# mistralai/mistral-inference

Measured on NVIDIA H100. Metric: decode tokens/sec (bf16, batch=1, seq=4k) [+ prefill TFLOPS, both vs roofline], higher is better.
Workload: dtype bf16

## Files before the change

mistral_inference_b200/csrc/abi.cu:

```cuda
#include <cmath>
#include <cstdlib>
#include <cstring>

#include "attn_decode_tma.cuh"
#include "attn_full_hd64.cuh"
#include "attn_prefill.cuh"
#include "attn_prefill_wgmma.cuh"
#include "decode_megakernel.cuh"
#include "elementwise.cuh"
#include "gemm_mma.cuh"
#include "gemm_streamk.cuh"
#include "gemm_wgmma.cuh"
#include "kv_fp8.cuh"
#include "lora.cuh"
#include "moe.cuh"
#include "sampling.cuh"
#include "skinny_linear.cuh"
#include "vision.cuh"
#include "workspace.cuh"

namespace mb200 {
thread_local char g_err[512] = "";
thread_local bool g_launch_log_on = false;
thread_local bool g_launch_log_overflow = false;
// ... 854 lines not shown
  MB_CHECK_ARG((size_t)sms * sizeof(unsigned long long) <= kWsMkArgmaxSlots.bytes, "decode_step: %d SMs exceed the argmax slots", sms);
  uint8_t* ws = (uint8_t*)workspace;
  p.argmax_counter = (int*)(ws + kWsMkArgmaxCounter.offset);
  p.argmax_slots = (unsigned long long*)(ws + kWsMkArgmaxSlots.offset);
  p.bar_flags = (unsigned*)(ws + kWsMkBarFlags.offset);
  p.bar_epoch = (unsigned*)(ws + kWsMkBarEpoch.offset);
  p.done_counter = (int*)(ws + kWsMkDoneCounter.offset);
  const DecodeScratch sc = decode_scratch(dim, hidden, n_heads, n_experts, top_k, sms);
  p.xbuf = (bf16*)(ws + sc.xbuf);
  p.hbuf = (bf16*)(ws + sc.hbuf);
  p.qbuf = (bf16*)(ws + sc.qbuf);
  p.abuf = (bf16*)(ws + sc.abuf);
  p.gbuf = (bf16*)(ws + sc.gbuf);
  p.partial = (float*)(ws + sc.partial);
  p.prof = g_mk_prof;
  p.prof_bar = g_mk_prof_bar;
  if (workspace_bytes < sc.end) return fail(MB200_E_WORKSPACE, "decode_step: workspace %zu < %zu", workspace_bytes, sc.end);

  void* args[] = {(void*)&p};
  const void* fn = nullptr;
  switch (rep) {
    case 1: fn = w8 ? (const void*)decode_megakernel<1, true> : (const void*)decode_megakernel<1>; break;
    case 2: fn = w8 ? (const void*)decode_megakernel<2, true> : (const void*)decode_megakernel<2>; break;
    case 4: fn = w8 ? (const void*)decode_megakernel<4, true> : (const void*)decode_megakernel<4>; break;
    case 6: fn = w8 ? (const void*)decode_megakernel<6, true> : (const void*)decode_megakernel<6>; break;
    case 8: fn = w8 ? (const void*)decode_megakernel<8, true> : (const void*)decode_megakernel<8>; break;
    default: return fail(MB200_E_INVALID, "decode_step: H/KV=%d unsupported (1,2,4,6,8)", rep);
  }
  if (w8)
    note_launch("decode_megakernel<%d, true>", rep);
  else
    note_launch("decode_megakernel<%d>", rep);
  MB_CHECK_CUDA(cudaFuncSetAttribute(fn, cudaFuncAttributeMaxDynamicSharedMemorySize, (int)smem));
  MB_CHECK_CUDA(cudaLaunchCooperativeKernel(fn, dim3((unsigned)sms), dim3(MK_THREADS), args, smem, (cudaStream_t)stream));
  return MB200_OK;
}

extern "C" {

int mb200_decode_step(const mb200_layer_desc* layers_dev, const int32_t* windows_dev, int64_t n_layers, const void* emb, const void* final_norm,
                      const void* w_out, const float* rope, const int64_t* token_dev, int64_t pos, int64_t batch_row, float* logits,
                      int64_t* next_token_dev, int64_t dim,
                      int64_t hidden, int64_t n_heads, int64_t n_kv_heads, int64_t head_dim, int64_t vocab, float eps, int64_t n_experts,
                      int64_t top_k, const void* const* moe_gate_dev, const void* const* moe_w13_dev, const void* const* moe_w2_dev,
                      void* workspace, size_t workspace_bytes, void* stream) {
  return decode_step_impl(layers_dev, windows_dev, n_layers, emb, final_norm, w_out, rope, token_dev, pos, batch_row, logits, next_token_dev, dim,
                          hidden, n_heads, n_kv_heads, head_dim, vocab, eps, n_experts, top_k, moe_gate_dev, moe_w13_dev, moe_w2_dev, workspace,
                          workspace_bytes, stream, false);
}

int mb200_decode_step_fp8(const mb200_layer_desc_fp8* layers_dev, const int32_t* windows_dev, int64_t n_layers, const void* emb,
                          const void* final_norm, const void* w_out, const float* rope, const int64_t* token_dev, int64_t pos,
                          int64_t batch_row, float* logits, int64_t* next_token_dev, int64_t dim, int64_t hidden, int64_t n_heads,
                          int64_t n_kv_heads, int64_t head_dim, int64_t vocab, float eps, void* workspace, size_t workspace_bytes, void* stream) {
  return decode_step_impl(layers_dev, windows_dev, n_layers, emb, final_norm, w_out, rope, token_dev, pos, batch_row, logits, next_token_dev, dim,
                          hidden, n_heads, n_kv_heads, head_dim, vocab, eps, 0, 0, nullptr, nullptr, nullptr, workspace, workspace_bytes, stream,
                          true);
}

int mb200_decode_step_fp8_supported(int64_t dim, int64_t hidden, int64_t n_heads, int64_t n_kv_heads, int64_t head_dim, int64_t vocab,
                                    int64_t smem_optin) {
  if (smem_optin <= 0) {
    int dev = 0, smem_max = 0;
    MB_CHECK_CUDA(cudaGetDevice(&dev));
    MB_CHECK_CUDA(cudaDeviceGetAttribute(&smem_max, cudaDevAttrMaxSharedMemoryPerBlockOptin, dev));
    smem_optin = smem_max;
  }
  DecodePlan plan;
  return decode_plan(dim, hidden, n_heads, n_kv_heads, head_dim, vocab, 0, 0, smem_optin, &plan, true);
}

int mb200_debug_decode_scratch(int64_t dim, int64_t hidden, int64_t n_heads, int64_t n_kv_heads, int64_t head_dim, int64_t n_experts,
                               int64_t top_k, size_t* q_offset, size_t* attn_offset) {
  MB_CHECK_ARG(q_offset && attn_offset, "debug_decode_scratch: null pointer");
  size_t off[6];
  const int rc = mb200_debug_decode_buffers(dim, hidden, n_heads, n_kv_heads, head_dim, n_experts, top_k, off);
  if (rc) return rc;
  *q_offset = off[2];
  *attn_offset = off[3];
  return MB200_OK;
}

int mb200_debug_decode_buffers(int64_t dim, int64_t hidden, int64_t n_heads, int64_t n_kv_heads, int64_t head_dim, int64_t n_experts,
                               int64_t top_k, size_t* offsets) {
  MB_CHECK_ARG(offsets, "debug_decode_buffers: null pointer");
  MB_CHECK_ARG(head_dim == kHeadDim && n_kv_heads > 0 && n_heads % n_kv_heads == 0 && dim > 0 && hidden > 0,
               "debug_decode_scratch: bad shape (H=%lld, KV=%lld, hd=%lld)", (long long)n_heads, (long long)n_kv_heads, (long long)head_dim);
  const DecodeScratch sc = decode_scratch(dim, hidden, n_heads, n_experts, top_k, 0);
  offsets[0] = sc.xbuf;
  offsets[1] = sc.hbuf;
  offsets[2] = sc.qbuf;
  offsets[3] = sc.abuf;
  offsets[4] = sc.gbuf;
  offsets[5] = sc.partial;
  return MB200_OK;
}

int mb200_decode_step_supported(int64_t dim, int64_t hidden, int64_t n_heads, int64_t n_kv_heads, int64_t head_dim, int64_t vocab,
                                int64_t n_experts, int64_t top_k, int64_t smem_optin) {
  if (smem_optin <= 0) {
    int dev = 0, smem_max = 0;
    MB_CHECK_CUDA(cudaGetDevice(&dev));
    MB_CHECK_CUDA(cudaDeviceGetAttribute(&smem_max, cudaDevAttrMaxSharedMemoryPerBlockOptin, dev));
    smem_optin = smem_max;
  }
  DecodePlan plan;
  return decode_plan(dim, hidden, n_heads, n_kv_heads, head_dim, vocab, n_experts, top_k, smem_optin, &plan);
}

int mb200_debug_set_decode_timeline(void* device_buffer) {
  g_mk_prof = (unsigned long long*)device_buffer;
  return MB200_OK;
}
int mb200_debug_set_barrier_timeline(void* device_buffer) {
  g_mk_prof_bar = (unsigned long long*)device_buffer;
  return MB200_OK;
}

int mb200_debug_launch_log(int enable, char* out, size_t out_bytes) {
  const bool overflow = g_launch_log_overflow;
  const size_t len = g_launch_log_len;
  g_launch_log_on = enable != 0;
  g_launch_log_overflow = false;
  g_launch_log_len = 0;
  if (out != nullptr) {
    if (out_bytes < len + 1) return fail(MB200_E_INVALID, "launch log: %zu bytes recorded, buffer of %zu", len, out_bytes);
    memcpy(out, g_launch_log, len);
    out[len] = '\0';
  }
  if (overflow) return fail(MB200_E_INVALID, "launch log: more than %zu bytes of launches since the last read", kLaunchLogBytes);
  return MB200_OK;
}

int mb200_test_gemm_naive(const void* a, const void* w, float* c, int64_t T, int64_t N, int64_t K, void* stream) {
  MB_CHECK_ARG(a && w && c, "test_gemm_naive: null pointer");
  const dim3 grid((unsigned)ceil_div(N, 128), (unsigned)T);
  gemm_naive_kernel<<<grid, 128, 0, (cudaStream_t)stream>>>((const bf16*)a, (const bf16*)w, c, (int)T, (int)N, (int)K);
  MB_CHECK_LAUNCH("gemm_naive_kernel");
  return MB200_OK;
}

}

#ifdef MB200_SK_TRACE
extern "C" int mb200_debug_sk_trace(void* host_out, size_t bytes, unsigned* count) {
  using namespace mb200;
  if (bytes < sizeof(sk_trace_buf)) return fail(MB200_E_INVALID, "sk trace: %zu < %zu", bytes, sizeof(sk_trace_buf));
  MB_CHECK_CUDA(cudaDeviceSynchronize());
  MB_CHECK_CUDA(cudaMemcpyFromSymbol(host_out, sk_trace_buf, sizeof(sk_trace_buf)));
  MB_CHECK_CUDA(cudaMemcpyFromSymbol(count, sk_trace_count, sizeof(unsigned)));
  return MB200_OK;
}
#endif
```

mistral_inference_b200/csrc/decode_megakernel.cuh:

```cuda
#pragma once
#include "common.cuh"
#include "gemm_mma.cuh"

namespace mb200 {

constexpr int MK_CONSUMER_WARPS = 8;
constexpr int MK_CONSUMERS = MK_CONSUMER_WARPS * 32;
constexpr int MK_PRODUCER_WARPS = 2;
constexpr int MK_THREADS = MK_CONSUMERS + 32 * MK_PRODUCER_WARPS;
constexpr int MK_WEIGHT_STAGE_BYTES = 16 * 1024;
constexpr int MK_MAX_KC = MK_WEIGHT_STAGE_BYTES / 4;
constexpr int MK_MAX_KC8 = MK_WEIGHT_STAGE_BYTES / 2;
constexpr int MK_KV_PAD = 16;
constexpr int MK_STAGE_BYTES = 16 * 1024 + 16 * MK_KV_PAD;
constexpr int MK_MAX_STAGES = 12;
constexpr int MK_MAX_SPLITS = 32;

struct MkLayer {
  const bf16* wqkv;
  const bf16* wo;
  const bf16* w13;
  const bf16* w2;
  const bf16* attn_norm;
  const bf16* ffn_norm;
// ... 210 lines not shown
};

enum : int { SEG_QKV, SEG_KV, SEG_WO, SEG_UP, SEG_DOWN };

template <bool W8 = false>
struct Walk {
  uint32_t it;
  int layer, seg, e, s, n;
  MatCut c;
  bool w8;
  int k_begin, k_end, pps;
  const bf16* W;
  const bf16* V;

  __device__ __forceinline__ bool done(const MkParams& p) const { return layer > p.n_layers; }
  __device__ __forceinline__ bool gated(const MkParams& p, int routed) const {
    return p.n_experts != 0 && layer < p.n_layers && seg == SEG_UP && e == 0 && routed != layer;
  }
  __device__ __forceinline__ void matrix(const bf16* w, int N, int K, bool e4m3 = false) {
    W = w;
    w8 = e4m3;
    c = cut_matrix(N, K, e4m3);
    n = matrix_stages(c, e4m3);
  }
  __device__ __forceinline__ int experts(const MkParams& p) const { return (seg == SEG_DOWN && p.n_experts) ? p.top_k : 1; }
  __device__ __forceinline__ void setup(const MkParams& p, uint32_t sel) {
    const int q_dim = p.H * kHeadDim, kv_dim = p.KV * kHeadDim;
    s = 0;
    if (layer == p.n_layers) {
      matrix(p.w_out, p.vocab, p.dim);
      return;
    }
    const MkLayer& L = W8 ? reinterpret_cast<const MkLayerFp8*>(p.layers)[layer].w : p.layers[layer];
    if (seg == SEG_QKV) {
      matrix(L.wqkv, q_dim + 2 * kv_dim, p.dim, W8);
    } else if (seg == SEG_KV) {
      const int win = p.windows[layer];
      const AttnSlice a = attn_slice(p, win);
      k_begin = a.k_begin;
      k_end = a.k_end;
      pps = a.pps;
      n = 2 * a.n_kvst;
      W = L.cache_k + ((int64_t)p.batch_row * win) * kv_dim;
      V = L.cache_v + ((int64_t)p.batch_row * win) * kv_dim;
    } else if (seg == SEG_WO) {
      matrix(L.wo, p.dim, q_dim, W8);
    } else if (seg == SEG_UP) {
      matrix(p.n_experts ? p.moe_w13[layer * p.n_experts + ((sel >> (8 * e)) & 0xff)] : L.w13, 2 * p.hidden, p.dim, W8);
    } else {
      matrix(L.w2, p.dim, p.hidden, W8);
      n *= experts(p);
    }
  }
  __device__ __forceinline__ void next_segment(const MkParams& p) {
    if (layer == p.n_layers) {
      ++layer;
      return;
    }
    if (seg == SEG_UP && ++e < (p.n_experts ? p.top_k : 1)) return;
    e = 0;
    if (++seg > SEG_DOWN) {
      seg = SEG_QKV;
      ++layer;
    }
  }
  __device__ __forceinline__ void settle(const MkParams& p, uint32_t sel, int routed) {
    for (;;) {
      n = 0;
      if (done(p) || gated(p, routed)) return;
      setup(p, sel);
      if (n > 0) return;
      next_segment(p);
    }
  }
  __device__ __forceinline__ void next(const MkParams& p, uint32_t sel, int routed) {
    ++it;
    if (++s < n) return;
    next_segment(p);
    settle(p, sel, routed);
  }

  __device__ __forceinline__ StageCopy stage(const MkParams& p, uint32_t sel) const {
    StageCopy sc;
    if (seg == SEG_KV) {
      const int64_t row_elems = (int64_t)p.KV * kHeadDim;
      const int k0 = k_begin + (s >> 1) * pps;
      sc.src = ((s & 1) ? V : W) + (int64_t)k0 * row_elems;
      sc.src_step = row_elems;
      sc.bytes = (uint32_t)row_elems * 2;
      sc.dst_step = sc.bytes + MK_KV_PAD;
      sc.count = min(pps, k_end - k0);
      return sc;
    }
    const int ne = experts(p), K = c.kc * c.nch;
    const int per_group = MK_CONSUMER_WARPS * c.nch * ne;
    const int gi = s / per_group, r = s - gi * per_group;
    const int g0 = c.p0 + gi * MK_CONSUMER_WARPS, g = min(MK_CONSUMER_WARPS, c.p1 - g0);
    const int j = r / (c.nch * g), r2 = r - j * (c.nch * g);
    const int ch = r2 / g, w = r2 - ch * g;
    const bf16* m = (seg == SEG_DOWN && p.n_experts) ? p.moe_w2[layer * p.n_experts + ((sel >> (8 * j)) & 0xff)] : W;
    if (W8 && w8 && two_pairs_per_stage(c, true)) {
      constexpr int kStagesPerGroup = MK_CONSUMER_WARPS / 2;
      const int g0 = c.p0 + (s / kStagesPerGroup) * MK_CONSUMER_WARPS, first = g0 + 2 * (s % kStagesPerGroup);
      sc.src = m + (int64_t)first * K;
      sc.src_step = 0;
      sc.bytes = (uint32_t)(min(2, c.p1 - first) * 2 * c.kc);
      sc.dst_step = 0;
      sc.count = 1;
      return sc;
    }
    if (W8 && w8) {
      const bf16* r8 = m + (int64_t)(g0 + w) * K;
      sc.bytes = (uint32_t)c.kc;
      sc.src = r8 + ((c.nch == 1) ? 0 : ch * (c.kc >> 1));
      sc.src_step = K >> 1;
      sc.dst_step = sc.bytes;
      sc.count = 2;
      if (c.nch == 1) {
        sc.bytes *= 2;
        sc.count = 1;
      }
      return sc;
    }
    const bf16* r0 = m + (int64_t)(2 * (g0 + w)) * K;
    sc.bytes = (uint32_t)c.kc * 2;
    if (c.nch == 1) {
      sc.src = r0;
      sc.src_step = 0;
      sc.bytes *= 2;
      sc.dst_step = 0;
      sc.count = 1;
    } else {
      sc.src = r0 + ch * c.kc;
      sc.src_step = K;
      sc.dst_step = sc.bytes;
      sc.count = 2;
    }
    return sc;
  }
};

__device__ __forceinline__ void bulk_g2s_hint(void* smem_dst, const void* gsrc, uint32_t bytes, uint64_t* bar, uint64_t policy) {
  asm volatile("cp.async.bulk.shared::cluster.global.mbarrier::complete_tx::bytes.L2::cache_hint [%0], [%1], %2, [%3], %4;" ::"r"(
                   smem_u32(smem_dst)),
               "l"(gsrc), "r"(bytes), "r"(smem_u32(bar)), "l"(policy)
               : "memory");
}
__device__ __forceinline__ unsigned long long globaltimer() {
  unsigned long long t;
  asm volatile("mov.u64 %0, %globaltimer;" : "=l"(t));
  return t;
}

constexpr int MK_INFLIGHT_CAP = 5;
static_assert(MK_INFLIGHT_CAP <= MK_CONSUMER_WARPS, "below the smallest ring decode_plan accepts (n_stages > MK_CONSUMER_WARPS)");
template <bool W8 = false>
struct Producer {
  uint8_t* ring;
  uint64_t* full;
  uint64_t* empty;
  int n_stages;
  uint64_t policy;
  int me;
  uint32_t slot, par;
  uint32_t cslot, cpar;
  uint32_t sel;
  int routed;
  unsigned long long* prof;

  __device__ __forceinline__ bool owns(uint32_t it) const { return (int)(it % (uint32_t)MK_PRODUCER_WARPS) == me; }
  __device__ __forceinline__ void advance(uint32_t it) {
    if (++slot == (uint32_t)n_stages) {
      slot = 0;
      par ^= 1;
    }
    if (it + 1 > (uint32_t)MK_INFLIGHT_CAP && ++cslot == (uint32_t)n_stages) {
      cslot = 0;
      cpar ^= 1;
    }
  }

  __device__ __forceinline__ void copy(const MkParams& p, const Walk<W8>& cp) {
    bool landed = cp.it < (uint32_t)MK_INFLIGHT_CAP || mbar_try_wait(&full[cslot], cpar);
    if (!landed || !mbar_try_wait(&empty[slot], par ^ 1)) {
      const unsigned long long t0 = prof != nullptr ? globaltimer() : 0ull;
      unsigned long long t_landed = t0;
      for (uint32_t spins = 0;;) {
        if (!landed && mbar_try_wait(&full[cslot], cpar)) {
          landed = true;
          if (prof != nullptr) t_landed = globaltimer();
        }
        if (landed && mbar_try_wait(&empty[slot], par ^ 1)) break;
        if (++spins == MB200_WATCHDOG_SPINS) __trap();
      }
      if (prof != nullptr) {
        const unsigned long long full_ns = globaltimer() - t_landed;
        unsigned long long* row = prof + (int64_t)min(cp.layer, p.n_layers - 1) * MK_PROF_WORDS + MK_PROF_STAMPS;
        row[me] += full_ns;
        row[2 + me] += t_landed - t0;
        if (full_ns >= MK_PROF_LONG_NS) row[4 + me] += full_ns;
      }
    }
    const StageCopy sc = cp.stage(p, sel);
    uint64_t* bar = &full[slot];
    mbar_arrive_expect_tx(bar, sc.bytes * (uint32_t)sc.count);
    uint8_t* dst = ring + (size_t)slot * MK_STAGE_BYTES;
    for (int r = 0; r < sc.count; ++r) bulk_g2s_hint(dst + r * sc.dst_step, sc.src + r * sc.src_step, sc.bytes, bar, policy);
  }
};

template <bool W8 = false>
__device__ __forceinline__ void producer_main(const MkParams& p, uint8_t* ring, uint64_t* full, uint64_t* empty, int me, const MoeRoute* route,
                                              uint64_t* route_bar) {
  Producer<W8> pr;
  pr.ring = ring;
  pr.full = full;
  pr.empty = empty;
  pr.n_stages = p.n_stages;
  pr.me = me;
  pr.slot = pr.par = pr.cslot = pr.cpar = 0;
  pr.sel = 0;
  pr.routed = -1;
  pr.prof = (p.prof != nullptr && blockIdx.x % 21 == 0) ? p.prof + (int64_t)(blockIdx.x / 21) * p.n_layers * MK_PROF_WORDS : nullptr;
  asm volatile("createpolicy.fractional.L2::evict_first.b64 %0, 1.0;" : "=l"(pr.policy));
  Walk<W8> cp;
  cp.it = 0;
  cp.layer = cp.seg = cp.e = 0;
  cp.settle(p, pr.sel, pr.routed);
  while (!cp.done(p)) {
    if (cp.n == 0) {
      mbar_wait(route_bar, (uint32_t)(cp.layer & 1), 8, (uint32_t)cp.layer);
      uint32_t sel = 0;
      for (int j = 0; j < p.top_k; ++j) sel |= (uint32_t)route->e[j] << (8 * j);
      pr.sel = sel;
      pr.routed = cp.layer;
      cp.settle(p, pr.sel, pr.routed);
      continue;
    }
    if (pr.owns(cp.it)) pr.copy(p, cp);
    pr.advance(cp.it);
    cp.next(p, pr.sel, pr.routed);
  }
}

__device__ __forceinline__ void consume_pair_stage(const uint8_t* ring, uint64_t* full, uint64_t* empty, int n_stages, uint32_t it,
                                                   const uint4* xc, int kc8, int lane, float& a0, float& a1) {
  const uint32_t slot = it % n_stages, par = (it / n_stages) & 1;
  mbar_wait(&empty[slot], par ^ 1, 2, it);
  mbar_wait(&full[slot], par, 3, it);
  const uint4* w0 = reinterpret_cast<const uint4*>(ring + (size_t)slot * MK_STAGE_BYTES);
  const uint4* w1 = w0 + kc8;
#pragma unroll 4
  for (int i = lane; i < kc8; i += 32) {
    const uint4 a = w0[i], b = w1[i], x = xc[i];
    const uint32_t aw[4] = {a.x, a.y, a.z, a.w}, bw[4] = {b.x, b.y, b.z, b.w}, xw[4] = {x.x, x.y, x.z, x.w};
#pragma unroll
    for (int j = 0; j < 4; ++j) {
      const float xl = bf16lo(xw[j]), xh = bf16hi(xw[j]);
      a0 = fmaf(bf16lo(aw[j]), xl, a0);
      a0 = fmaf(bf16hi(aw[j]), xh, a0);
      a1 = fmaf(bf16lo(bw[j]), xl, a1);
      a1 = fmaf(bf16hi(bw[j]), xh, a1);
    }
  }
  __syncwarp();
  if (lane == 0) mbar_arrive_n(&empty[slot], MK_CONSUMER_WARPS);
}

__device__ __forceinline__ void consume_pair_stage_w8(const uint8_t* ring, uint64_t* full, uint64_t* empty, int n_stages, uint32_t it,
                                                      const uint4* xc, int kq, int row0, uint32_t arrivals, int lane, float& a0, float& a1) {
  const uint32_t slot = it % n_stages, par = (it / n_stages) & 1;
  mbar_wait(&empty[slot], par ^ 1, 2, it);
  mbar_wait(&full[slot], par, 3, it);
  const uint4* w0 = reinterpret_cast<const uint4*>(ring + (size_t)slot * MK_STAGE_BYTES) + row0;
  const uint4* w1 = w0 + kq;
#pragma unroll 2
  for (int i = lane; i < kq; i += 32) {
    const uint4 a = w0[i], b = w1[i];
    const uint32_t aq[4] = {a.x, a.y, a.z, a.w}, bq[4] = {b.x, b.y, b.z, b.w};
#pragma unroll
    for (int h = 0; h < 2; ++h) {
      const uint4 x = xc[2 * i + h];
      const uint32_t xw[4] = {x.x, x.y, x.z, x.w};
#pragma unroll
      for (int j = 0; j < 4; ++j) {
        const float2 af = e4m3x2_to_float2(aq[2 * h + (j >> 1)] >> (16 * (j & 1)));
        const float2 bf = e4m3x2_to_float2(bq[2 * h + (j >> 1)] >> (16 * (j & 1)));
        const float xl = bf16lo(xw[j]), xh = bf16hi(xw[j]);
        a0 = fmaf(af.x, xl, a0);
        a0 = fmaf(af.y, xh, a0);
        a1 = fmaf(bf.x, xl, a1);
        a1 = fmaf(bf.y, xh, a1);
      }
    }
  }
  __syncwarp();
  if (lane == 0) mbar_arrive_n(&empty[slot], arrivals);
}

template <bool W8 = false, class Pre, class Epi>
__device__ __forceinline__ void consume_matrix(int N, int K, const uint8_t* ring, uint64_t* full, uint64_t* empty, int n_stages, RingState& rs,
                                               const uint4* xs, int tid, Pre pre, Epi epi, const float* wscale = nullptr) {
  const MatCut c = cut_matrix(N, K, W8);
  const bool two = two_pairs_per_stage(c, W8);
  const int lane = tid & 31, warp = tid >> 5;
  const int kc8 = c.kc >> 3;
  for (int g0 = c.p0; g0 < c.p1; g0 += MK_CONSUMER_WARPS) {
// ... 540 lines not shown
```

mistral_inference_b200/csrc/gemm_wgmma.cuh:

```cuda
#pragma once
#include <cuda.h>
#include <cuda_fp16.h>
#include <cuda_fp8.h>

#include <cstdlib>

#include "decode_megakernel.cuh"
#include "epilogue.cuh"
#include "gemm_mma.cuh"
#include "wgmma.cuh"

namespace mb200 {

constexpr int TG_BM = 128, TG_BN = 256, TG_BK = 64;
template <int BN, int TA = 128, bool W8 = false>
struct TgCfg {
  static constexpr int kABytes = TA * TG_BK * 2;
  static constexpr int kBBytes = BN * TG_BK * 2;
  static constexpr int kRawBytes = W8 ? BN * TG_BK : 0;
  static constexpr int kStageBytes = kABytes + kBBytes + kRawBytes;
  static constexpr int kWG = TA > 64 ? 2 : 1;
  static constexpr int kThreads = 128 * (1 + kWG);
  static constexpr int kSlack = kStageBytes < 64 * TG_BK * 2 ? 64 * TG_BK * 2 - kStageBytes : 0;
  static constexpr int kMaxStages = (227 * 1024 - 1024 - 512 - kSlack) / kStageBytes;
  static constexpr int kShortRingStages = ((W8 ? 200 : 100) * 1024) / kStageBytes;
  static constexpr int kStages = (TA < 128 || BN < 128) ? (kShortRingStages < 3 ? 3 : (kShortRingStages > kMaxStages ? kMaxStages : kShortRingStages))
                                                        : W8 ? kMaxStages : (BN == 128 ? 6 : 4);
  static constexpr int kSmem = kStages * kStageBytes + kSlack + 1024  + 512 ;
  static_assert(kSmem <= 227 * 1024, "shared memory plan exceeds the 227 KB of an sm_90 block");
};

struct TcGemmParams {
  int T, N, K;
  EpiParams epi;
};

__device__ __forceinline__ void tma_load_2d(void* smem_dst, const CUtensorMap* map, uint64_t* bar, int c0, int c1) {
  asm volatile("cp.async.bulk.tensor.2d.shared::cluster.global.mbarrier::complete_tx::bytes [%0], [%1, {%3, %4}], [%2];" ::"r"(smem_u32(smem_dst)),
               "l"(map), "r"(smem_u32(bar)), "r"(c0), "r"(c1)
               : "memory");
}
__device__ __forceinline__ void tma_load_2d_multicast(void* smem_dst, const CUtensorMap* map, uint64_t* bar, int c0, int c1, uint16_t cta_mask) {
  asm volatile(
      "cp.async.bulk.tensor.2d.shared::cluster.global.mbarrier::complete_tx::bytes.multicast::cluster [%0], [%1, {%3, %4}], [%2], %5;" ::"r"(
          smem_u32(smem_dst)),
      "l"(map), "r"(smem_u32(bar)), "r"(c0), "r"(c1), "h"(cta_mask)
      : "memory");
}
__device__ __forceinline__ uint32_t cluster_ctarank() {
  uint32_t r;
  asm volatile("mov.u32 %0, %%cluster_ctarank;" : "=r"(r));
  return r;
}
__device__ __forceinline__ void cluster_sync_all() {
  asm volatile("barrier.cluster.arrive.release.aligned;" ::: "memory");
  asm volatile("barrier.cluster.wait.acquire.aligned;" ::: "memory");
}
__device__ __forceinline__ void mbar_arrive_cluster(uint64_t* bar, uint32_t cta) {
  uint32_t remote;
  asm volatile("mapa.shared::cluster.u32 %0, %1, %2;" : "=r"(remote) : "r"(smem_u32(bar)), "r"(cta));
  asm volatile("mbarrier.arrive.release.cluster.shared::cluster.b64 _, [%0];" ::"r"(remote) : "memory");
}

constexpr int W8_CONVERTERS = 96;
template <int BN, bool DENSE = false>
__device__ __forceinline__ void convert_w8_tile(const uint8_t* raw, uint8_t* wtile, const float* __restrict__ scale_rows, int ct) {
#pragma unroll 2
  for (int q = ct; q < BN * (TG_BK / 16); q += W8_CONVERTERS) {
    const int row = q >> 2, c = q & 3;
    const uint4 v = *reinterpret_cast<const uint4*>(raw + row * TG_BK + c * 16);
    const uint32_t in[4] = {v.x, v.y, v.z, v.w};
    uint32_t o[8];
    if constexpr (DENSE) {
#pragma unroll
      for (int j = 0; j < 8; ++j) {
        const float2 f = e4m3x2_to_float2(in[j >> 1] >> (16 * (j & 1)));
        o[j] = pack2_rn(f.x, f.y);
      }
    } else {
    const float s = __ldg(scale_rows + row);
#pragma unroll
    for (int j = 0; j < 8; ++j) {
      const __half2_raw hr = __nv_cvt_fp8x2_to_halfraw2((__nv_fp8x2_storage_t)(in[j >> 1] >> (16 * (j & 1))), __NV_E4M3);
      const float2 f = __half22float2(*reinterpret_cast<const __half2*>(&hr));
      const __nv_bfloat162 b = __floats2bfloat162_rn(__fmul_rn(f.x, s), __fmul_rn(f.y, s));
      o[j] = *reinterpret_cast<const uint32_t*>(&b);
    }
    }
    uint8_t* dst = wtile + row * (TG_BK * 2);
    *reinterpret_cast<uint4*>(dst + (((2 * c) ^ (row & 7)) << 4)) = make_uint4(o[0], o[1], o[2], o[3]);
    *reinterpret_cast<uint4*>(dst + (((2 * c + 1) ^ (row & 7)) << 4)) = make_uint4(o[4], o[5], o[6], o[7]);
  }
  asm volatile("fence.proxy.async.shared::cta;" ::: "memory");
}

template <int BN>
__device__ __forceinline__ void wgmma_kblock(float (&acc)[BN / 2], uint32_t a_addr, uint32_t b_addr, bool first) {
  const uint64_t adesc = wgmma_desc_sw128(a_addr), bdesc = wgmma_desc_sw128(b_addr);
  wgmma_fence();
#pragma unroll
  for (int k = 0; k < TG_BK / 16; ++k)
    wgmma_ss(acc, adesc + (uint64_t)(2 * k), bdesc + (uint64_t)(2 * k), (first && k == 0) ? 0u : 1u);
  wgmma_commit();
}

template <int MODE, int BN>
__device__ __forceinline__ void epi_fragment(const EpiParams& epi, const float (&acc)[BN / 2], int t0, int n0, int lane, int limit) {
  const int nc = n0 + 2 * (lane & 3);
#pragma unroll
  for (int j = 0; j < BN / 8; ++j) {
    if (t0 < limit) epi_pair<MODE>(epi, t0, nc + 8 * j, acc[4 * j], acc[4 * j + 1]);
    if (t0 + 8 < limit) epi_pair<MODE>(epi, t0 + 8, nc + 8 * j, acc[4 * j + 2], acc[4 * j + 3]);
  }
}

constexpr int MOE_PLAN_HEADER = 64;
constexpr int MOE_PAIR_SECOND = 1 << 30;
constexpr int MOE_MAX_EXPERTS = 16;
struct MoeWeightMaps {
  CUtensorMap m[MOE_MAX_EXPERTS];
};
struct MoeWeightScales {
  const float* s[MOE_MAX_EXPERTS];
};

template <int MODE, int CL, int BN, int TA, bool GROUPED, bool W8 = false>
__device__ __forceinline__ void tc_gemm_body(const CUtensorMap& map_a, const CUtensorMap* map_w_base, const TcGemmParams& p, const int32_t* plan,
                                             const MoeWeightScales* scales = nullptr) {
  static_assert(TA == 128 || CL == 1, "small-batch variant is single-CTA");
  static_assert(!W8 || CL == 1, "FP8 weights: single-CTA variant only");
  static_assert(!W8 || GROUPED || (MODE & EPI_WSCALE) != 0, "FP8 dense weights: the epilogue applies the row scales");
  using Cfg = TgCfg<BN, TA, W8>;
  constexpr int STAGES = Cfg::kStages, B_BYTES = Cfg::kBBytes, STAGE_BYTES = Cfg::kStageBytes, A_BYTES = Cfg::kABytes;
  extern __shared__ uint8_t smem_raw[];
  uint8_t* smem = reinterpret_cast<uint8_t*>((reinterpret_cast<uintptr_t>(smem_raw) + 1023) & ~(uintptr_t)1023);
  uint64_t* full = reinterpret_cast<uint64_t*>(smem + STAGES * STAGE_BYTES + Cfg::kSlack);
  uint64_t* empty = full + STAGES;
  uint64_t* raw = empty + STAGES;

  const int warp = threadIdx.x >> 5, lane = threadIdx.x & 31;
  const int rank = CL > 1 ? (int)cluster_ctarank() : 0;
  const int cta = (int)blockIdx.x / CL, n_cta = (int)gridDim.x / CL;
  const int num_m = GROUPED ? (CL > 1 ? plan[6] : plan[0]) : ((p.T + TG_BM - 1) / TG_BM + CL - 1) / CL;
  const int num_n = p.N / BN, num_tiles = num_m * num_n, num_k = p.K / TG_BK;
  const int32_t* tile_expert = GROUPED ? plan + MOE_PLAN_HEADER + (CL > 1 ? 2 * plan[2] : 0) : nullptr;
  const int32_t* tile_row0 = GROUPED ? tile_expert + plan[2] : nullptr;
  constexpr int kGM = CL > 1 ? 8 : 12, kGN = CL > 1 ? 9 : 12;
  auto tile_mn = [&](int tile, int& mu, int& nt) {
    if (num_m <= 16) {
      mu = tile % num_m;
      nt = tile / num_m;
      return;
    }
    const int per_row = kGN * num_m, rows_full = num_n / kGN;
    int nb, r, gn;
    if (tile < rows_full * per_row) {
      nb = tile / per_row;
      r = tile % per_row;
      gn = kGN;
    } else {
      nb = rows_full;
      r = tile - rows_full * per_row;
      gn = num_n - rows_full * kGN;
    }
    const int blk = kGM * gn, mb_full = num_m / kGM;
    int mblk, q, gm;
    if (r < mb_full * blk) {
      mblk = r / blk;
      q = r % blk;
      gm = kGM;
    } else {
      mblk = mb_full;
      q = r - mb_full * blk;
      gm = num_m - mb_full * kGM;
    }
    mu = mblk * kGM + q % gm;
    nt = nb * kGN + q / gm;
  };
  auto grouped_m0 = [&](int u, bool& store) {
    const int info = tile_row0[u];
    store = true;
    if (CL == 1) return info;
    const int row0 = info & (MOE_PAIR_SECOND - 1);
    if (rank == 0) return row0;
    store = (info & MOE_PAIR_SECOND) != 0;
    return store ? row0 + TG_BM : row0;
  };
  const CUtensorMap& map_w = *map_w_base;

  if (threadIdx.x == 0) {
    for (int i = 0; i < STAGES; ++i) {
      mbar_init(&full[i], W8 ? 1 + W8_CONVERTERS : 1);
      mbar_init(&empty[i], CL * Cfg::kWG);
      if (W8) mbar_init(&raw[i], 1);
    }
    asm volatile("fence.mbarrier_init.release.cluster;" ::: "memory");
    asm volatile("prefetch.tensormap [%0];" ::"l"(&map_a) : "memory");
    if (!GROUPED) asm volatile("prefetch.tensormap [%0];" ::"l"(&map_w) : "memory");
  }
  if (CL > 1)
    cluster_sync_all();
  else
    __syncthreads();

  if (warp == 0) {
    if (lane == 0) {
      uint32_t it = 0;
      for (int tile = cta; tile < num_tiles; tile += n_cta) {
        bool store_unused;
        int mu, nt;
        tile_mn(tile, mu, nt);
        const int m0 = GROUPED ? grouped_m0(mu, store_unused) : (mu * CL + rank) * TG_BM, n0 = nt * BN;
        const CUtensorMap* wmap = GROUPED ? map_w_base + tile_expert[mu] : map_w_base;
        for (int kb = 0; kb < num_k; ++kb, ++it) {
          const uint32_t s = it % STAGES, par = (it / STAGES) & 1;
          mbar_wait_quiet(&empty[s], par ^ 1);
          uint8_t* sa = smem + s * STAGE_BYTES;
          if constexpr (W8) {
            mbar_arrive_expect_tx(&full[s], A_BYTES);
            tma_load_2d(sa, &map_a, &full[s], kb * TG_BK, m0);
            mbar_arrive_expect_tx(&raw[s], Cfg::kRawBytes);
            tma_load_2d(sa + A_BYTES + B_BYTES, wmap, &raw[s], kb * TG_BK, n0);
            continue;
          }
          mbar_arrive_expect_tx(&full[s], STAGE_BYTES);
          tma_load_2d(sa, &map_a, &full[s], kb * TG_BK, m0);
          if (CL > 1)
            tma_load_2d_multicast(sa + A_BYTES + rank * (B_BYTES / CL), wmap, &full[s], kb * TG_BK, n0 + rank * (BN / CL),
                                  (uint16_t)((1u << CL) - 1));
          else
            tma_load_2d(sa + A_BYTES, wmap, &full[s], kb * TG_BK, n0);
        }
      }
    }
  } else if (W8 && warp < 4) {
    const int ct = (int)threadIdx.x - 32;
    uint32_t it = 0;
    for (int tile = cta; tile < num_tiles; tile += n_cta) {
      int mu, nt;
      tile_mn(tile, mu, nt);
      const float* srows = GROUPED ? scales->s[tile_expert[mu]] + nt * BN : nullptr;
      for (int kb = 0; kb < num_k; ++kb, ++it) {
        const uint32_t s = it % STAGES, par = (it / STAGES) & 1;
        mbar_wait_quiet(&raw[s], par);
        uint8_t* sa = smem + s * STAGE_BYTES;
        convert_w8_tile<BN, !GROUPED>(sa + A_BYTES + B_BYTES, sa + A_BYTES, srows, ct);
        mbar_arrive(&full[s]);
      }
    }
  } else if (warp >= 4) {
    const int wg = (warp >> 2) - 1, wt = (int)threadIdx.x & 127;
    const int row_in_tile = wg * 64 + ((warp & 3) << 4) + (lane >> 2);
    auto release = [&](uint32_t s) {
      if (wt == 0) {
        if (CL > 1) {
          for (uint32_t c = 0; c < (uint32_t)CL; ++c) mbar_arrive_cluster(&empty[s], c);
        } else {
          mbar_arrive(&empty[s]);
        }
      }
    };
    uint32_t it = 0;
    float acc[BN / 2];
    for (int tile = cta; tile < num_tiles; tile += n_cta) {
      bool store = true;
      int mu, nt;
      tile_mn(tile, mu, nt);
      const int m0 = GROUPED ? grouped_m0(mu, store) : (mu * CL + rank) * TG_BM, n0 = nt * BN;
      for (int kb = 0; kb < num_k; ++kb, ++it) {
        const uint32_t s = it % STAGES, par = (it / STAGES) & 1;
        mbar_wait_quiet(&full[s], par);
        const uint32_t a_addr = smem_u32(smem + s * STAGE_BYTES) + wg * 64 * TG_BK * 2;
        wgmma_kblock<BN>(acc, a_addr, smem_u32(smem + s * STAGE_BYTES) + A_BYTES, kb == 0);
        if (kb > 0) {
          wgmma_wait<1>();
          release((it - 1) % STAGES);
        }
      }
      wgmma_wait<0>();
      wgmma_fence_acc(acc);
      release((it - 1) % STAGES);
      const int limit = store ? min(p.T, m0 + TA) : 0;
      epi_fragment<MODE, BN>(p.epi, acc, m0 + row_in_tile, n0, lane, limit);
    }
  }
  if (CL > 1) cluster_sync_all();
}

template <int MODE, int CL, int BN, int TA = 128>
__global__ void __launch_bounds__(TgCfg<BN, TA>::kThreads, 1)
    gemm_wgmma_kernel(const __grid_constant__ CUtensorMap map_a, const __grid_constant__ CUtensorMap map_w, const TcGemmParams p) {
  tc_gemm_body<MODE, CL, BN, TA, false>(map_a, &map_w, p, nullptr);
}

template <int MODE, int CL, int BN, int TA>
__global__ void __launch_bounds__(TgCfg<BN, TA>::kThreads, 1)
    gemm_wgmma_grouped_kernel(const __grid_constant__ CUtensorMap map_a, const __grid_constant__ MoeWeightMaps maps_w, const TcGemmParams p,
                              const int32_t* __restrict__ plan) {
  tc_gemm_body<MODE, CL, BN, TA, true>(map_a, maps_w.m, p, plan);
}

template <int MODE, int BN, int TA>
__global__ void __launch_bounds__(TgCfg<BN, TA, true>::kThreads, 1)
    gemm_wgmma_fp8_kernel(const __grid_constant__ CUtensorMap map_a, const __grid_constant__ CUtensorMap map_w, const TcGemmParams p) {
  tc_gemm_body<MODE, 1, BN, TA, false, true>(map_a, &map_w, p, nullptr);
}

template <int MODE, int BN, int TA>
__global__ void __launch_bounds__(TgCfg<BN, TA, true>::kThreads, 1)
    gemm_wgmma_grouped_fp8_kernel(const __grid_constant__ CUtensorMap map_a, const __grid_constant__ MoeWeightMaps maps_w,
                                  const __grid_constant__ MoeWeightScales scales, const TcGemmParams p, const int32_t* __restrict__ plan) {
  tc_gemm_body<MODE, 1, BN, TA, true, true>(map_a, maps_w.m, p, plan, &scales);
}

typedef CUresult (*PFN_encodeTiled)(CUtensorMap*, CUtensorMapDataType, cuuint32_t, void*, const cuuint64_t*, const cuuint64_t*, const cuuint32_t*,
                                    const cuuint32_t*, CUtensorMapInterleave, CUtensorMapSwizzle, CUtensorMapL2promotion, CUtensorMapFloatOOBfill);

inline PFN_encodeTiled get_encode_tiled() {
  static PFN_encodeTiled fn = nullptr;
  if (fn == nullptr) {
    void* ptr = nullptr;
    cudaDriverEntryPointQueryResult qres;
    if (cudaGetDriverEntryPoint("cuTensorMapEncodeTiled", &ptr, cudaEnableDefault, &qres) == cudaSuccess && qres == cudaDriverEntryPointSuccess)
      fn = reinterpret_cast<PFN_encodeTiled>(ptr);
  }
  return fn;
}

inline int make_tensor_map_2d(CUtensorMap* map, const void* base, int64_t rows, int64_t K, int box_rows) {
  PFN_encodeTiled enc = get_encode_tiled();
  if (enc == nullptr) return fail(MB200_E_CUDA, "cuTensorMapEncodeTiled entry point not available");
  const cuuint64_t dims[2] = {(cuuint64_t)K, (cuuint64_t)rows};
  const cuuint64_t strides[1] = {(cuuint64_t)K * 2};
  const cuuint32_t box[2] = {(cuuint32_t)TG_BK, (cuuint32_t)box_rows};
  const cuuint32_t estr[2] = {1, 1};
  const CUresult r = enc(map, CU_TENSOR_MAP_DATA_TYPE_BFLOAT16, 2, const_cast<void*>(base), dims, strides, box, estr, CU_TENSOR_MAP_INTERLEAVE_NONE,
                         CU_TENSOR_MAP_SWIZZLE_128B, CU_TENSOR_MAP_L2_PROMOTION_L2_256B, CU_TENSOR_MAP_FLOAT_OOB_FILL_NONE);
  if (r != CUDA_SUCCESS) return fail(MB200_E_CUDA, "cuTensorMapEncodeTiled failed (%d) rows=%lld K=%lld", (int)r, (long long)rows, (long long)K);
  return MB200_OK;
}

inline int make_tensor_map_e4m3(CUtensorMap* map, const void* base, int64_t rows, int64_t K, int box_rows) {
  PFN_encodeTiled enc = get_encode_tiled();
  if (enc == nullptr) return fail(MB200_E_CUDA, "cuTensorMapEncodeTiled entry point not available");
  const cuuint64_t dims[2] = {(cuuint64_t)K, (cuuint64_t)rows};
  const cuuint64_t strides[1] = {(cuuint64_t)K};
  const cuuint32_t box[2] = {(cuuint32_t)TG_BK, (cuuint32_t)box_rows};
  const cuuint32_t estr[2] = {1, 1};
  const CUresult r = enc(map, CU_TENSOR_MAP_DATA_TYPE_UINT8, 2, const_cast<void*>(base), dims, strides, box, estr, CU_TENSOR_MAP_INTERLEAVE_NONE,
                         CU_TENSOR_MAP_SWIZZLE_NONE, CU_TENSOR_MAP_L2_PROMOTION_L2_256B, CU_TENSOR_MAP_FLOAT_OOB_FILL_NONE);
  if (r != CUDA_SUCCESS) return fail(MB200_E_CUDA, "cuTensorMapEncodeTiled (e4m3) failed (%d) rows=%lld K=%lld", (int)r, (long long)rows, (long long)K);
  return MB200_OK;
}

inline bool wgmma_gemm_eligible(int64_t T, int64_t N, int64_t K) {
  if (K % TG_BK != 0) return false;
  if (T >= TG_BM) return N % 128 == 0 || N % 192 == 0;
  return N % 32 == 0;
}

inline bool wgmma_cluster_enabled() {
  const char* e = getenv("MB200_GEMM_CLUSTER");
  return !(e != nullptr && e[0] == '0');
}
inline int wgmma_forced_bn() {
  const char* e = getenv("MB200_GEMM_BN");
  return e != nullptr ? atoi(e) : 0;
}

template <int MODE, int BN>
int launch_gemm_wgmma_bn(const GemmParams& g, bool pair, int sms, cudaStream_t stream) {
  using Cfg = TgCfg<BN>;
  CUtensorMap map_a, map_w;
  int rc = make_tensor_map_2d(&map_a, g.a, g.T, g.K, TG_BM);
  if (rc) return rc;
  rc = make_tensor_map_2d(&map_w, g.w, g.N, g.K, pair ? BN / 2 : BN);
  if (rc) return rc;
  TcGemmParams p;
  p.T = g.T;
  p.N = g.N;
  p.K = g.K;
  p.epi = g.epi;
  if (pair) {
    const int supers = ceil_div(ceil_div(g.T, TG_BM), 2) * (g.N / BN), pairs = sms / 2;
    MB_CHECK_CUDA(cudaFuncSetAttribute(gemm_wgmma_kernel<MODE, 2, BN>, cudaFuncAttributeMaxDynamicSharedMemorySize, Cfg::kSmem));
    cudaLaunchConfig_t cfg = {};
    cfg.gridDim = dim3(2u * (unsigned)(supers < pairs ? supers : pairs));
    cfg.blockDim = dim3(Cfg::kThreads);
    cfg.dynamicSmemBytes = Cfg::kSmem;
    cfg.stream = stream;
    cudaLaunchAttribute at[1];
    at[0].id = cudaLaunchAttributeClusterDimension;
    at[0].val.clusterDim.x = 2;
    at[0].val.clusterDim.y = 1;
    at[0].val.clusterDim.z = 1;
    cfg.attrs = at;
    cfg.numAttrs = 1;
    MB_CHECK_CUDA(cudaLaunchKernelEx(&cfg, gemm_wgmma_kernel<MODE, 2, BN>, map_a, map_w, p));
    note_launch("gemm_wgmma_kernel<%d, 2, %d, %d>", MODE, BN, TG_BM);
    MB_CHECK_LAUNCH("gemm_wgmma_kernel<cluster 2>");
    return MB200_OK;
  }
  const int tiles = ceil_div(g.T, TG_BM) * (g.N / BN);
  MB_CHECK_CUDA(cudaFuncSetAttribute(gemm_wgmma_kernel<MODE, 1, BN>, cudaFuncAttributeMaxDynamicSharedMemorySize, Cfg::kSmem));
  gemm_wgmma_kernel<MODE, 1, BN><<<tiles < sms ? tiles : sms, Cfg::kThreads, Cfg::kSmem, stream>>>(map_a, map_w, p);
  note_launch("gemm_wgmma_kernel<%d, 1, %d, %d>", MODE, BN, TG_BM);
  MB_CHECK_LAUNCH("gemm_wgmma_kernel");
  return MB200_OK;
}

inline int wgmma_small_bn(int64_t N, int sms) {
  const int forced = wgmma_forced_bn();
  if ((forced == 32 || forced == 64 || forced == 128 || forced == 256) && N % forced == 0) return forced;
  int best = 0;
  double best_score = -1.0;
  const int cand[4] = {256, 128, 64, 32};
  for (int i = 0; i < 4; ++i) {
    const int bn = cand[i];
    if (N % bn != 0) continue;
    const int64_t tiles = N / bn, rounds = (tiles + sms - 1) / sms;
    double score = (double)tiles / (double)(rounds * sms);
    if (tiles < sms / 2) score *= 0.5;
    if (score > best_score + 1e-9) {
      best_score = score;
      best = bn;
    }
  }
  return best;
}

template <int MODE, int BN, int TA>
int launch_gemm_wgmma_small_bn(const GemmParams& g, int sms, cudaStream_t stream) {
  using Cfg = TgCfg<BN, TA>;
  CUtensorMap map_a, map_w;
  int rc = make_tensor_map_2d(&map_a, g.a, g.T, g.K, TA);
  if (rc) return rc;
// ... 101 lines not shown
```

Before: 184.1.

## Add wgmma GEMM trace probes, relax cluster arrive ordering, lower decode in-flight cap

```diff
diff --git a/mistral_inference_b200/csrc/abi.cu b/mistral_inference_b200/csrc/abi.cu
--- a/mistral_inference_b200/csrc/abi.cu
+++ b/mistral_inference_b200/csrc/abi.cu
@@ -1030,3 +1030,17 @@
   return MB200_OK;
 }
 #endif
+
+#ifdef MB200_TC_TRACE
+extern "C" int mb200_debug_tc_trace(void* host_out, size_t bytes) {
+  using namespace mb200;
+  if (host_out != nullptr && bytes < sizeof(tc_trace_buf)) return fail(MB200_E_INVALID, "tc trace: %zu < %zu", bytes, sizeof(tc_trace_buf));
+  MB_CHECK_CUDA(cudaDeviceSynchronize());
+  if (host_out != nullptr) MB_CHECK_CUDA(cudaMemcpyFromSymbol(host_out, tc_trace_buf, sizeof(tc_trace_buf)));
+  void* dev = nullptr;
+  MB_CHECK_CUDA(cudaGetSymbolAddress(&dev, tc_trace_buf));
+  MB_CHECK_CUDA(cudaMemset(dev, 0, sizeof(tc_trace_buf)));
+  MB_CHECK_CUDA(cudaDeviceSynchronize());
+  return MB200_OK;
+}
+#endif
diff --git a/mistral_inference_b200/csrc/decode_megakernel.cuh b/mistral_inference_b200/csrc/decode_megakernel.cuh
--- a/mistral_inference_b200/csrc/decode_megakernel.cuh
+++ b/mistral_inference_b200/csrc/decode_megakernel.cuh
@@ -386,7 +386,7 @@
   return t;
 }
 
-constexpr int MK_INFLIGHT_CAP = 5;
+constexpr int MK_INFLIGHT_CAP = 4;
 static_assert(MK_INFLIGHT_CAP <= MK_CONSUMER_WARPS, "below the smallest ring decode_plan accepts (n_stages > MK_CONSUMER_WARPS)");
 template <bool W8 = false>
 struct Producer {
diff --git a/mistral_inference_b200/csrc/gemm_wgmma.cuh b/mistral_inference_b200/csrc/gemm_wgmma.cuh
--- a/mistral_inference_b200/csrc/gemm_wgmma.cuh
+++ b/mistral_inference_b200/csrc/gemm_wgmma.cuh
@@ -59,7 +59,7 @@
 __device__ __forceinline__ void mbar_arrive_cluster(uint64_t* bar, uint32_t cta) {
   uint32_t remote;
   asm volatile("mapa.shared::cluster.u32 %0, %1, %2;" : "=r"(remote) : "r"(smem_u32(bar)), "r"(cta));
-  asm volatile("mbarrier.arrive.release.cluster.shared::cluster.b64 _, [%0];" ::"r"(remote) : "memory");
+  asm volatile("mbarrier.arrive.shared::cluster.b64 _, [%0];" ::"r"(remote) : "memory");
 }
 
 constexpr int W8_CONVERTERS = 96;
@@ -94,6 +94,26 @@
   asm volatile("fence.proxy.async.shared::cta;" ::: "memory");
 }
 
+#ifdef MB200_TC_TRACE
+constexpr int TC_TRACE_CTAS = 160, TC_TRACE_TILES = 64, TC_TRACE_POINTS = 4;
+__device__ unsigned long long tc_trace_buf[TC_TRACE_CTAS][TC_TRACE_TILES][TC_TRACE_POINTS][2];
+__device__ __forceinline__ void tc_now(unsigned long long& g, unsigned long long& c) {
+  asm volatile("mov.u64 %0, %%globaltimer;" : "=l"(g));
+  asm volatile("mov.u64 %0, %%clock64;" : "=l"(c));
+}
+__device__ __forceinline__ void tc_trace_put(int tile_i, int point, unsigned long long g, unsigned long long c) {
+  if (blockIdx.x < TC_TRACE_CTAS && tile_i < TC_TRACE_TILES) {
+    tc_trace_buf[blockIdx.x][tile_i][point][0] = g;
+    tc_trace_buf[blockIdx.x][tile_i][point][1] = c;
+  }
+}
+__device__ __forceinline__ void tc_stamp(int tile_i, int point) {
+  unsigned long long g, c;
+  tc_now(g, c);
+  tc_trace_put(tile_i, point, g, c);
+}
+#endif
+
 template <int BN>
 __device__ __forceinline__ void wgmma_kblock(float (&acc)[BN / 2], uint32_t a_addr, uint32_t b_addr, bool first) {
   const uint64_t adesc = wgmma_desc_sw128(a_addr), bdesc = wgmma_desc_sw128(b_addr);
@@ -206,15 +226,31 @@
   if (warp == 0) {
     if (lane == 0) {
       uint32_t it = 0;
+#ifdef MB200_TC_TRACE
+      int tile_i = 0;
+#endif
       for (int tile = cta; tile < num_tiles; tile += n_cta) {
         bool store_unused;
         int mu, nt;
         tile_mn(tile, mu, nt);
         const int m0 = GROUPED ? grouped_m0(mu, store_unused) : (mu * CL + rank) * TG_BM, n0 = nt * BN;
         const CUtensorMap* wmap = GROUPED ? map_w_base + tile_expert[mu] : map_w_base;
+#ifdef MB200_TC_TRACE
+        unsigned long long stall_g = 0, stall_c = 0;
+#endif
         for (int kb = 0; kb < num_k; ++kb, ++it) {
           const uint32_t s = it % STAGES, par = (it / STAGES) & 1;
+#ifdef MB200_TC_TRACE
+          unsigned long long g0, c0, g1, c1;
+          tc_now(g0, c0);
           mbar_wait_quiet(&empty[s], par ^ 1);
+          tc_now(g1, c1);
+          stall_g += g1 - g0;
+          stall_c += c1 - c0;
+          if (kb == num_k - 1) tc_trace_put(tile_i++, 3, stall_g, stall_c);
+#else
+          mbar_wait_quiet(&empty[s], par ^ 1);
+#endif
           uint8_t* sa = smem + s * STAGE_BYTES;
           if constexpr (W8) {
             mbar_arrive_expect_tx(&full[s], A_BYTES);
@@ -262,6 +298,10 @@
     };
     uint32_t it = 0;
     float acc[BN / 2];
+#ifdef MB200_TC_TRACE
+    int tile_i = 0;
+    const bool tracer = (int)threadIdx.x == 128;
+#endif
     for (int tile = cta; tile < num_tiles; tile += n_cta) {
       bool store = true;
       int mu, nt;
@@ -270,6 +310,9 @@
       for (int kb = 0; kb < num_k; ++kb, ++it) {
         const uint32_t s = it % STAGES, par = (it / STAGES) & 1;
         mbar_wait_quiet(&full[s], par);
+#ifdef MB200_TC_TRACE
+        if (tracer && kb == 0) tc_stamp(tile_i, 0);
+#endif
         const uint32_t a_addr = smem_u32(smem + s * STAGE_BYTES) + wg * 64 * TG_BK * 2;
         wgmma_kblock<BN>(acc, a_addr, smem_u32(smem + s * STAGE_BYTES) + A_BYTES, kb == 0);
         if (kb > 0) {
@@ -279,9 +322,16 @@
       }
       wgmma_wait<0>();
       wgmma_fence_acc(acc);
+#ifdef MB200_TC_TRACE
+      if (tracer) tc_stamp(tile_i, 1);
+#endif
       release((it - 1) % STAGES);
       const int limit = store ? min(p.T, m0 + TA) : 0;
       epi_fragment<MODE, BN>(p.epi, acc, m0 + row_in_tile, n0, lane, limit);
+#ifdef MB200_TC_TRACE
+      if (tracer) tc_stamp(tile_i, 2);
+      ++tile_i;
+#endif
     }
   }
   if (CL > 1) cluster_sync_all();
```

Result: faster. 186.8, median of 6 (+1.4%).
